# volume-em/empanada

Measured on AMD Instinct MI355X. Metric: Mvox/s end-to-end 3D panoptic inference (incl. consensus); PQ vs CPU ref, higher is better.
Workload: dtype f32

## Files before the change

empanada_amd/csrc/emp_wino4.hip:

```cpp
#include "emp_common.h"
#include "emp_wino4.h"
#include <stdlib.h>
#include <type_traits>

typedef float f32x4 __attribute__((ext_vector_type(4)));

#define WF_THREADS 512
#define WF_G 32
#define WF_S 16
#define WF_RS 34
#define WF_PS (WF_S * WF_RS)
#define WF_PF 3
#define WF_XCH (WF_THREADS * 48)
#define WF_T_MIN 3136

struct WfGeom {
    const float *x, *U, *scale, *shift;
    const int32_t *tiles;
    float *out;
    int64_t T, out_ps;
    int H, W, dil, groups;
};

template <int CIN, int COUT, bool RELU>
__global__ __launch_bounds__(WF_THREADS, 2) void wino4_fused_kernel(WfGeom g)
{
    constexpr int KS = CIN / WF_S;
    constexpr int CG = COUT / 64;
    __shared__ __attribute__((aligned(16))) float Vs[36 * WF_PS > WF_XCH ? 36 * WF_PS : WF_XCH];

    const int tid = threadIdx.x, wave = tid >> 6, lane = tid & 63;
    const int tl = tid >> 4, ch = tid & 15;
    const int ci = lane & 15, q = lane >> 4;
    const int odd = q >> 1;
    const int h = wave >> 2, w4 = wave & 3;

    const int xcd = blockIdx.x & 7, slot = blockIdx.x >> 3, per = gridDim.x >> 3;
    const int lo = (int)((int64_t)g.groups * xcd / 8), hi = (int)((int64_t)g.groups * (xcd + 1) / 8);
    const int n_items = slot < hi - lo ? ((hi - lo - slot + per - 1) / per) * CG : 0;

    auto load_raw = [&](int item, int s, v1 (&raw)[6][6]) -> int {
        const int64_t t = (int64_t)(lo + slot + (item / CG) * per) * WF_G + tl;
        const bool live = t < g.T;
        const int64_t tc = live ? t : g.T - 1;
        const int n = g.tiles[3 * tc], by = g.tiles[3 * tc + 1], bx = g.tiles[3 * tc + 2];
        const uint32_t src = 4u * ((uint32_t)n * (uint32_t)(g.H * g.W * CIN) + (uint32_t)(WF_S * s + ch));
        const char *xb = reinterpret_cast<const char *>(g.x);
        int mask = 0;
        uint32_t xo[6];
#pragma unroll
        for (int b = 0; b < 6; ++b) {
            const int xx = bx + b * g.dil;
            if (live && xx >= 0 && xx < g.W) mask |= 64 << b;
            xo[b] = 4u * (uint32_t)(min(max(xx, 0), g.W - 1) * CIN);
        }
#pragma unroll
        for (int a = 0; a < 6; ++a) {
            const int yy = by + a * g.dil;
            if (live && yy >= 0 && yy < g.H) mask |= 1 << a;
            const uint32_t row = src + 4u * (uint32_t)(min(max(yy, 0), g.H - 1) * (g.W * CIN));
#pragma unroll
            for (int b = 0; b < 6; ++b) raw[a][b] = {*reinterpret_cast<const float *>(xb + (row + xo[b]))};
        }
        return mask;
    };
    auto transform = [&](const v1 (&raw)[6][6], int mask) {
        v1 tt[6][6];
#pragma unroll
        for (int a = 0; a < 6; ++a) {
            v1 d[6];
#pragma unroll
            for (int b = 0; b < 6; ++b) d[b] = {(mask >> a & 1) && (mask >> (6 + b) & 1) ? raw[a][b].x : 0.f};
            wino4_bt(d, tt[a]);
        }
        float *dst = &Vs[ch * WF_RS + tl];
#pragma unroll
        for (int v = 0; v < 6; ++v) {
            v1 col[6], r[6];
#pragma unroll
            for (int a = 0; a < 6; ++a) col[a] = tt[a][v];
            wino4_bt(col, r);
#pragma unroll
            for (int u = 0; u < 6; ++u) dst[(u * 6 + v) * WF_PS] = r[u].x;
        }
    };

    const float *Al = &Vs[3 * h * WF_PS + (8 * (q & 1) + odd) * WF_RS + ci];
    const float *Ul = g.U + ((int64_t)3 * h * COUT + 16 * w4 + ci) * CIN + 8 * (q & 1) + 4 * odd;

    v1 raw[6][6];
    int mask = 0;
    if (n_items > 0) mask = load_raw(0, 0, raw);
    for (int item = 0; item < n_items; ++item) {
        const int cg = item % CG;
        f32x4 acc[18][2];
#pragma unroll
        for (int lp = 0; lp < 18; ++lp)
#pragma unroll
            for (int rt = 0; rt < 2; ++rt) acc[lp][rt] = {0.f, 0.f, 0.f, 0.f};

#pragma unroll 1
        for (int s = 0; s < KS; ++s) {
            transform(raw, mask);
            __syncthreads();
            const float *up = Ul + (int64_t)cg * 64 * CIN + WF_S * s;
            auto uoff = [](int lp) { return (int64_t)((lp / 3) * 6 + lp % 3) * COUT * CIN; };
            float4 bq[WF_PF];
#pragma unroll
            for (int lp = 0; lp < WF_PF; ++lp) bq[lp] = *reinterpret_cast<const float4 *>(up + uoff(lp));
            if (s + 1 < KS) mask = load_raw(item, s + 1, raw);
#pragma unroll
            for (int lp = 0; lp < 18; ++lp) {
                float4 c = bq[lp % WF_PF];
                asm volatile("" : "+v"(c.x), "+v"(c.y), "+v"(c.z), "+v"(c.w));
                if (lp + WF_PF < 18) bq[lp % WF_PF] = *reinterpret_cast<const float4 *>(up + uoff(lp + WF_PF));
                const auto s0 = __builtin_amdgcn_permlane32_swap(__float_as_uint(c.x), __float_as_uint(c.y), false, false);
                const auto s1 = __builtin_amdgcn_permlane32_swap(__float_as_uint(c.z), __float_as_uint(c.w), false, false);
                const float bv[4] = {__uint_as_float(s0[0]), __uint_as_float(s1[0]), __uint_as_float(s0[1]), __uint_as_float(s1[1])};
                const float *ap = Al + ((lp / 3) * 6 + lp % 3) * WF_PS;
#pragma unroll
                for (int j = 0; j < 4; ++j)
#pragma unroll
                    for (int rt = 0; rt < 2; ++rt)
                        acc[lp][rt] = __builtin_amdgcn_mfma_f32_16x16x4f32(ap[2 * j * WF_RS + 16 * rt], bv[j], acc[lp][rt], 0, 0, 0);
            }
            __syncthreads();
        }

        const int co = cg * 64 + 16 * w4 + ci;
        float keep[4][3][4];
        float *xw = &Vs[((wave ^ 4) * 48) * 64 + lane];
        const float *xr = &Vs[(wave * 48) * 64 + lane];
        auto rows = [&](auto rtc, auto sendc) {
            constexpr int rt = decltype(rtc)::value;
            constexpr bool send = decltype(sendc)::value;
#pragma unroll
            for (int bb = 0; bb < 3; ++bb)
#pragma unroll
                for (int r = 0; r < 4; ++r) {
                    v1 m[6], rr[4];
#pragma unroll
                    for (int a = 0; a < 6; ++a) m[a] = {acc[3 * a + bb][rt][r]};
                    wino4_at(m, rr);
#pragma unroll
                    for (int a = 0; a < 4; ++a) {
                        if (send) xw[((r * 3 + bb) * 4 + a) * 64] = rr[a].x;
                        else keep[r][bb][a] = rr[a].x;
                    }
                }
        };
        using std::integral_constant;
        if (h == 0) {
            rows(integral_constant<int, 1>(), integral_constant<bool, true>());
            rows(integral_constant<int, 0>(), integral_constant<bool, false>());
        } else {
            rows(integral_constant<int, 0>(), integral_constant<bool, true>());
            rows(integral_constant<int, 1>(), integral_constant<bool, false>());
        }
        if (item + 1 < n_items) mask = load_raw(item + 1, 0, raw);
        __syncthreads();

        const float sc = g.scale[co], sh = g.shift[co];
        const int64_t t0 = (int64_t)(lo + slot + (item / CG) * per) * WF_G + 16 * h + 4 * q;
#pragma unroll
        for (int r = 0; r < 4; ++r) {
            const int64_t t = t0 + r;
            if (t < g.T) {
                const int n = g.tiles[3 * t], oy = g.tiles[3 * t + 1] + g.dil, ox = g.tiles[3 * t + 2] + g.dil;
                float *dst = g.out + (int64_t)n * g.H * g.W * g.out_ps + co;
#pragma unroll
                for (int a = 0; a < 4; ++a) {
                    v1 sm[6], yv[4];
#pragma unroll
                    for (int bb = 0; bb < 3; ++bb) {
                        const float got = xr[((r * 3 + bb) * 4 + a) * 64];
                        sm[bb] = {h ? got : keep[r][bb][a]};
                        sm[3 + bb] = {h ? keep[r][bb][a] : got};
                    }
                    wino4_at(sm, yv);
#pragma unroll
                    for (int b = 0; b < 4; ++b) {
                        const int yy = oy + a * g.dil, xx = ox + b * g.dil;
                        if (yy < g.H && xx < g.W) {
                            float v = __fadd_rn(__fmul_rn(yv[b].x, sc), sh);
                            if (RELU) v = fmaxf(v, 0.f);
                            dst[((int64_t)yy * g.W + xx) * g.out_ps] = v;
                        }
                    }
                }
            }
        }
        __syncthreads();
    }
}

static bool wf_off()
{
    static const char *off = getenv("EMP_WINO4_NO_FUSED");
    return off && off[0] == '1';
}

static bool wf_shape_ok(int64_t T, int Cin, int Cout)
{
    return ((Cin == 64 && Cout == 64) || (Cin == 128 && Cout == 128)) && T > 0 && 16 * T * Cin < (1LL << 30) &&
           emp_conv_k_slab(T, Cout, 36, 0) == WF_S;
}

extern "C" int emp_wino4_fused_eligible(int64_t T, int Cin, int Cout, int has_scale_shift)
{
    if (wf_off() || !has_scale_shift) return 0;
    if (!(Cin == 64 && Cout == 64)) return 0;
    return wf_shape_ok(T, Cin, Cout) && T >= WF_T_MIN;
}

extern "C" int emp_wino4_conv_bn_act_nhwc(const float *x, int N, int H, int W, int Cin, int dil, const int32_t *tiles,
                                          int64_t T, const float *U, int Cout, const float *scale, const float *shift,
                                          int relu, float *out, int64_t out_pixel_stride, void *stream)
{
    EMP_REQUIRE(x && tiles && U && scale && shift && out, "wino4_conv: null pointer (scale and shift are required)");
    EMP_REQUIRE(N > 0 && H > 0 && W > 0 && dil >= 1 && T >= 0, "wino4_conv: bad shape");
    if (out_pixel_stride == 0) out_pixel_stride = Cout;
    EMP_REQUIRE(out_pixel_stride >= Cout, "wino4_conv: bad pixel stride");
    EMP_REQUIRE(((reinterpret_cast<uintptr_t>(x) | reinterpret_cast<uintptr_t>(U)) & 15) == 0 &&
                (reinterpret_cast<uintptr_t>(out) & 3) == 0, "wino4_conv: alignment");
    if (T == 0) return EMP_OK;
    EMP_REQUIRE(wf_shape_ok(T, Cin, Cout), "wino4_conv: 64 -> 64 or 128 -> 128 with the K-slab 16 plan only (T = %lld, %d -> %d)",
                (long long)T, Cin, Cout);
    EMP_REQUIRE((int64_t)N * H * W * Cin < (1LL << 30) && T < (1LL << 31) - WF_G, "wino4_conv: activation too large for 32-bit byte offsets");
    WfGeom g;
    g.x = x; g.U = U; g.scale = scale; g.shift = shift; g.tiles = tiles; g.out = out;
    g.T = T; g.out_ps = out_pixel_stride; g.H = H; g.W = W; g.dil = dil;
    g.groups = (int)emp_cdiv(T, WF_G);
    hipStream_t st = emp_stream(stream);
    const dim3 grid(256), block(WF_THREADS);
    if (Cin == 64) {
        if (relu) hipLaunchKernelGGL((wino4_fused_kernel<64, 64, true>), grid, block, 0, st, g);
        else hipLaunchKernelGGL((wino4_fused_kernel<64, 64, false>), grid, block, 0, st, g);
    } else {
        if (relu) hipLaunchKernelGGL((wino4_fused_kernel<128, 128, true>), grid, block, 0, st, g);
        else hipLaunchKernelGGL((wino4_fused_kernel<128, 128, false>), grid, block, 0, st, g);
    }
    EMP_CHECK_LAUNCH("emp_wino4_conv_bn_act_nhwc");
    return EMP_OK;
}
```

Baseline: 133.1.

## Stage Winograd input gathers through LDS with async global_load_lds and deeper U prefetch

Replaces the register-held raw input gather with global_load_lds_dword writes into a new LDS staging area, issued row by row during the MFMA loop of the previous slab. Filter (U) loads use inline-asm global_load_dwordx4 with a prefetch depth of 8 and explicit vmcnt waits computed per step, in place of the old depth-3 prefetch. Tile metadata and scale/shift loads for the epilogue and the next item are hoisted earlier, and one trailing barrier is removed. The aim is to hide global latency and cut register pressure, at the cost of a larger LDS footprint and fragile hand-counted vmcnt and m0 handling.

```diff
diff --git a/empanada_amd/csrc/emp_wino4.hip b/empanada_amd/csrc/emp_wino4.hip
--- a/empanada_amd/csrc/emp_wino4.hip
+++ b/empanada_amd/csrc/emp_wino4.hip
@@ -10,7 +10,8 @@
 #define WF_S 16
 #define WF_RS 34
 #define WF_PS (WF_S * WF_RS)
-#define WF_PF 3
+#define WF_UD 8
+#define WF_STG (WF_THREADS * 36)
 #define WF_XCH (WF_THREADS * 48)
 #define WF_T_MIN 3136
 
@@ -22,12 +23,59 @@
     int H, W, dil, groups;
 };
 
+__device__ __forceinline__ void wf_glds4(const char *sbase, uint32_t vrow, uint32_t vcol, unsigned lds_byte_addr)
+{
+    uint32_t voff;
+    asm volatile("v_add_u32 %0, %1, %2\n\ts_mov_b32 m0, %4\n\ts_nop 2\n\tglobal_load_lds_dword %0, %3"
+                 : "=&v"(voff) : "v"(vrow), "v"(vcol), "s"(sbase), "s"(lds_byte_addr) : "m0");
+}
+__device__ __forceinline__ f32x4 wf_ldu(const float *sbase, uint32_t voff)
+{
+    f32x4 r;
+    asm volatile("s_nop 4\n\tglobal_load_dwordx4 %0, %1, %2" : "=v"(r) : "v"(voff), "s"(sbase));
+    return r;
+}
+template <int N>
+__device__ __forceinline__ void wf_wait_u(f32x4 &c)
+{
+    asm volatile("s_waitcnt vmcnt(%1)" : "+v"(c) : "n"(N));
+}
+__device__ __forceinline__ void wf_wait_u(int n, f32x4 &c)
+{
+#define WF_W1(k) case k: wf_wait_u<k>(c); break;
+#define WF_W8(k) WF_W1(k) WF_W1(k + 1) WF_W1(k + 2) WF_W1(k + 3) WF_W1(k + 4) WF_W1(k + 5) WF_W1(k + 6) WF_W1(k + 7)
+    switch (n) {
+        WF_W8(0) WF_W8(8) WF_W8(16) WF_W8(24) WF_W8(32) WF_W8(40) WF_W8(48) WF_W8(56)
+        default: wf_wait_u<0>(c);
+    }
+#undef WF_W8
+#undef WF_W1
+}
+__device__ __forceinline__ void wf_wait_all()
+{
+    asm volatile("s_waitcnt vmcnt(0)" ::: "memory");
+}
+constexpr int wf_younger(int lp, bool gather)
+{
+    const int u = (lp + WF_UD - 1 < 17 ? lp + WF_UD - 1 : 17) - lp;
+    const int first = lp < WF_UD ? 0 : lp - WF_UD, last = lp - 1 < 5 ? lp - 1 : 5;
+    return u + (gather && last >= first ? 6 * (last - first + 1) : 0);
+}
+
 template <int CIN, int COUT, bool RELU>
 __global__ __launch_bounds__(WF_THREADS, 2) void wino4_fused_kernel(WfGeom g)
 {
     constexpr int KS = CIN / WF_S;
     constexpr int CG = COUT / 64;
-    __shared__ __attribute__((aligned(16))) float Vs[36 * WF_PS > WF_XCH ? 36 * WF_PS : WF_XCH];
+    static_assert(WF_XCH <= 36 * WF_PS + WF_STG && WF_UD >= 6 && WF_UD <= 18 && wf_younger(WF_UD, true) < 64, "LDS / vmcnt budget");
+    __shared__ __attribute__((aligned(16))) float Ls[WF_STG + 36 * WF_PS];
+    typedef __attribute__((address_space(3))) float lds_f;
+    auto fixed = [](float *p) {
+        unsigned a = (unsigned)(size_t)(lds_f *)p;
+        asm volatile("" : "+v"(a));
+        return (lds_f *)(size_t)a;
+    };
+    float *const Vs = Ls + WF_STG;
 
     const int tid = threadIdx.x, wave = tid >> 6, lane = tid & 63;
     const int tl = tid >> 4, ch = tid & 15;
@@ -39,41 +87,51 @@
     const int lo = (int)((int64_t)g.groups * xcd / 8), hi = (int)((int64_t)g.groups * (xcd + 1) / 8);
     const int n_items = slot < hi - lo ? ((hi - lo - slot + per - 1) / per) * CG : 0;
 
-    auto load_raw = [&](int item, int s, v1 (&raw)[6][6]) -> int {
-        const int64_t t = (int64_t)(lo + slot + (item / CG) * per) * WF_G + tl;
-        const bool live = t < g.T;
-        const int64_t tc = live ? t : g.T - 1;
-        const int n = g.tiles[3 * tc], by = g.tiles[3 * tc + 1], bx = g.tiles[3 * tc + 2];
-        const uint32_t src = 4u * ((uint32_t)n * (uint32_t)(g.H * g.W * CIN) + (uint32_t)(WF_S * s + ch));
-        const char *xb = reinterpret_cast<const char *>(g.x);
-        int mask = 0;
-        uint32_t xo[6];
+    uint32_t rowo[6], colo[6];
+    int mask = 0;
+    auto tile_geom = [&](int n, int by, int bx, bool live) {
+        const uint32_t src = 4u * ((uint32_t)n * (uint32_t)(g.H * g.W * CIN) + (uint32_t)ch);
+        mask = 0;
 #pragma unroll
         for (int b = 0; b < 6; ++b) {
             const int xx = bx + b * g.dil;
             if (live && xx >= 0 && xx < g.W) mask |= 64 << b;
-            xo[b] = 4u * (uint32_t)(min(max(xx, 0), g.W - 1) * CIN);
+            colo[b] = 4u * (uint32_t)(min(max(xx, 0), g.W - 1) * CIN);
         }
 #pragma unroll
         for (int a = 0; a < 6; ++a) {
             const int yy = by + a * g.dil;
             if (live && yy >= 0 && yy < g.H) mask |= 1 << a;
-            const uint32_t row = src + 4u * (uint32_t)(min(max(yy, 0), g.H - 1) * (g.W * CIN));
-#pragma unroll
-            for (int b = 0; b < 6; ++b) raw[a][b] = {*reinterpret_cast<const float *>(xb + (row + xo[b]))};
-        }
-        return mask;
-    };
-    auto transform = [&](const v1 (&raw)[6][6], int mask) {
+            rowo[a] = src + 4u * (uint32_t)(min(max(yy, 0), g.H - 1) * (g.W * CIN));
+        }
+    };
+    auto tile_index = [&](int item) -> int64_t {
+        const int64_t t = (int64_t)(lo + slot + (item / CG) * per) * WF_G + tl;
+        return t < g.T ? t : g.T - 1;
+    };
+    auto tile_live = [&](int item) { return (int64_t)(lo + slot + (item / CG) * per) * WF_G + tl < g.T; };
+    const unsigned lds0 = (unsigned)(size_t)(__attribute__((address_space(3))) float *)Ls;
+    const unsigned stg_dst = __builtin_amdgcn_readfirstlane(lds0 + (unsigned)(64 * wave * 4));
+    auto gather_row = [&](int a, int s) {
+        const char *xs = reinterpret_cast<const char *>(g.x) + 4 * WF_S * s;
+#pragma unroll
+        for (int b = 0; b < 6; ++b) wf_glds4(xs, rowo[a], colo[b], stg_dst + (unsigned)((a * 6 + b) * WF_THREADS * 4));
+    };
+    lds_f *const raw0 = fixed(&Ls[tid]), *const raw1 = fixed(&Ls[18 * WF_THREADS + tid]);
+    lds_f *const dst0 = fixed(&Vs[ch * WF_RS + tl]), *const dst1 = fixed(&Vs[18 * WF_PS + ch * WF_RS + tl]);
+    auto transform = [&]() {
         v1 tt[6][6];
 #pragma unroll
         for (int a = 0; a < 6; ++a) {
             v1 d[6];
-#pragma unroll
-            for (int b = 0; b < 6; ++b) d[b] = {(mask >> a & 1) && (mask >> (6 + b) & 1) ? raw[a][b].x : 0.f};
+            float val[6];
+#pragma unroll
+            for (int b = 0; b < 6; ++b) val[b] = (a < 3 ? raw0 : raw1)[((a % 3) * 6 + b) * WF_THREADS];
+            asm volatile("" : "+v"(val[0]), "+v"(val[1]), "+v"(val[2]), "+v"(val[3]), "+v"(val[4]), "+v"(val[5]));
+#pragma unroll
+            for (int b = 0; b < 6; ++b) d[b] = {(mask >> a & 1) && (mask >> (6 + b) & 1) ? val[b] : 0.f};
             wino4_bt(d, tt[a]);
         }
-        float *dst = &Vs[ch * WF_RS + tl];
 #pragma unroll
         for (int v = 0; v < 6; ++v) {
             v1 col[6], r[6];
@@ -81,16 +139,20 @@
             for (int a = 0; a < 6; ++a) col[a] = tt[a][v];
             wino4_bt(col, r);
 #pragma unroll
-            for (int u = 0; u < 6; ++u) dst[(u * 6 + v) * WF_PS] = r[u].x;
-        }
-    };
-
-    const float *Al = &Vs[3 * h * WF_PS + (8 * (q & 1) + odd) * WF_RS + ci];
-    const float *Ul = g.U + ((int64_t)3 * h * COUT + 16 * w4 + ci) * CIN + 8 * (q & 1) + 4 * odd;
-
-    v1 raw[6][6];
-    int mask = 0;
-    if (n_items > 0) mask = load_raw(0, 0, raw);
+            for (int u = 0; u < 6; ++u) (u < 3 ? dst0 : dst1)[((u % 3) * 6 + v) * WF_PS] = r[u].x;
+        }
+    };
+
+    lds_f *const Al0 = fixed(&Vs[3 * h * WF_PS + (8 * (q & 1) + odd) * WF_RS + ci]);
+    lds_f *const Al1 = fixed(&Vs[(18 + 3 * h) * WF_PS + (8 * (q & 1) + odd) * WF_RS + ci]);
+    const uint32_t uvo = 4u * (uint32_t)((3 * h * COUT + 16 * w4 + ci) * CIN + 8 * (q & 1) + 4 * odd);
+
+    if (n_items > 0) {
+        const int64_t tc = tile_index(0);
+        tile_geom(g.tiles[3 * tc], g.tiles[3 * tc + 1], g.tiles[3 * tc + 2], tile_live(0));
+#pragma unroll
+        for (int a = 0; a < 6; ++a) gather_row(a, 0);
+    }
     for (int item = 0; item < n_items; ++item) {
         const int cg = item % CG;
         f32x4 acc[18][2];
@@ -99,25 +161,26 @@
 #pragma unroll
             for (int rt = 0; rt < 2; ++rt) acc[lp][rt] = {0.f, 0.f, 0.f, 0.f};
 
-#pragma unroll 1
-        for (int s = 0; s < KS; ++s) {
-            transform(raw, mask);
+        auto slab = [&](int s, auto nextc) {
+            constexpr bool NEXT = decltype(nextc)::value;
+            wf_wait_all();
+            transform();
             __syncthreads();
-            const float *up = Ul + (int64_t)cg * 64 * CIN + WF_S * s;
-            auto uoff = [](int lp) { return (int64_t)((lp / 3) * 6 + lp % 3) * COUT * CIN; };
-            float4 bq[WF_PF];
-#pragma unroll
-            for (int lp = 0; lp < WF_PF; ++lp) bq[lp] = *reinterpret_cast<const float4 *>(up + uoff(lp));
-            if (s + 1 < KS) mask = load_raw(item, s + 1, raw);
+            const float *ub = g.U + (int64_t)cg * 64 * CIN + WF_S * s;
+            auto upos = [](int lp) { return (int64_t)((lp / 3) * 6 + lp % 3) * COUT * CIN; };
+            f32x4 bq[WF_UD];
+#pragma unroll
+            for (int lp = 0; lp < WF_UD; ++lp) bq[lp] = wf_ldu(ub + upos(lp), uvo);
 #pragma unroll
             for (int lp = 0; lp < 18; ++lp) {
-                float4 c = bq[lp % WF_PF];
-                asm volatile("" : "+v"(c.x), "+v"(c.y), "+v"(c.z), "+v"(c.w));
-                if (lp + WF_PF < 18) bq[lp % WF_PF] = *reinterpret_cast<const float4 *>(up + uoff(lp + WF_PF));
+                f32x4 c = bq[lp % WF_UD];
+                wf_wait_u(wf_younger(lp, NEXT), c);
+                if (lp + WF_UD < 18) bq[lp % WF_UD] = wf_ldu(ub + upos(lp + WF_UD), uvo);
+                if (NEXT && lp < 6) gather_row(lp, s + 1);
                 const auto s0 = __builtin_amdgcn_permlane32_swap(__float_as_uint(c.x), __float_as_uint(c.y), false, false);
                 const auto s1 = __builtin_amdgcn_permlane32_swap(__float_as_uint(c.z), __float_as_uint(c.w), false, false);
                 const float bv[4] = {__uint_as_float(s0[0]), __uint_as_float(s1[0]), __uint_as_float(s0[1]), __uint_as_float(s1[1])};
-                const float *ap = Al + ((lp / 3) * 6 + lp % 3) * WF_PS;
+                const lds_f *ap = (lp < 9 ? Al0 : Al1) + ((lp / 3 % 3) * 6 + lp % 3) * WF_PS;
 #pragma unroll
                 for (int j = 0; j < 4; ++j)
 #pragma unroll
@@ -125,12 +188,30 @@
                         acc[lp][rt] = __builtin_amdgcn_mfma_f32_16x16x4f32(ap[2 * j * WF_RS + 16 * rt], bv[j], acc[lp][rt], 0, 0, 0);
             }
             __syncthreads();
-        }
+        };
+        using std::integral_constant;
+#pragma unroll 1
+        for (int s = 0; s < KS - 1; ++s) slab(s, integral_constant<bool, true>());
+        slab(KS - 1, integral_constant<bool, false>());
 
         const int co = cg * 64 + 16 * w4 + ci;
+        const int64_t t0 = (int64_t)(lo + slot + (item / CG) * per) * WF_G + 16 * h + 4 * q;
+        const bool more = item + 1 < n_items, new_group = more && (item + 1) % CG == 0;
+        float sc, sh;
+        int on[4], oy[4], ox[4], nn, nby, nbx;
+        auto request = [&]() {
+            sc = g.scale[co], sh = g.shift[co];
+#pragma unroll
+            for (int r = 0; r < 4; ++r) {
+                const int64_t tc = t0 + r < g.T ? t0 + r : g.T - 1;
+                on[r] = g.tiles[3 * tc], oy[r] = g.tiles[3 * tc + 1], ox[r] = g.tiles[3 * tc + 2];
+            }
+            const int64_t tn = tile_index(item + 1);
+            nn = g.tiles[3 * tn], nby = g.tiles[3 * tn + 1], nbx = g.tiles[3 * tn + 2];
+        };
         float keep[4][3][4];
-        float *xw = &Vs[((wave ^ 4) * 48) * 64 + lane];
-        const float *xr = &Vs[(wave * 48) * 64 + lane];
+        float *xw = &Ls[((wave ^ 4) * 48) * 64 + lane];
+        const float *xr = &Ls[(wave * 48) * 64 + lane];
         auto rows = [&](auto rtc, auto sendc) {
             constexpr int rt = decltype(rtc)::value;
             constexpr bool send = decltype(sendc)::value;
@@ -149,38 +230,50 @@
                     }
                 }
         };
-        using std::integral_constant;
         if (h == 0) {
             rows(integral_constant<int, 1>(), integral_constant<bool, true>());
+            request();
             rows(integral_constant<int, 0>(), integral_constant<bool, false>());
         } else {
             rows(integral_constant<int, 0>(), integral_constant<bool, true>());
+            request();
             rows(integral_constant<int, 1>(), integral_constant<bool, false>());
         }
-        if (item + 1 < n_items) mask = load_raw(item + 1, 0, raw);
         __syncthreads();
-
-        const float sc = g.scale[co], sh = g.shift[co];
-        const int64_t t0 = (int64_t)(lo + slot + (item / CG) * per) * WF_G + 16 * h + 4 * q;
+        float got[4][3][4];
+#pragma unroll
+        for (int r = 0; r < 4; ++r)
+#pragma unroll
+            for (int bb = 0; bb < 3; ++bb)
+#pragma unroll
+                for (int a = 0; a < 4; ++a) got[r][bb][a] = xr[((r * 3 + bb) * 4 + a) * 64];
+        asm volatile("" : "+v"(sc), "+v"(sh), "+v"(nn), "+v"(nby), "+v"(nbx));
+#pragma unroll
+        for (int r = 0; r < 4; ++r) asm volatile("" : "+v"(on[r]), "+v"(oy[r]), "+v"(ox[r]));
+        __syncthreads();
+        if (more) {
+            if (new_group) tile_geom(nn, nby, nbx, tile_live(item + 1));
+#pragma unroll
+            for (int a = 0; a < 6; ++a) gather_row(a, 0);
+        }
+
 #pragma unroll
         for (int r = 0; r < 4; ++r) {
-            const int64_t t = t0 + r;
-            if (t < g.T) {
-                const int n = g.tiles[3 * t], oy = g.tiles[3 * t + 1] + g.dil, ox = g.tiles[3 * t + 2] + g.dil;
-                float *dst = g.out + (int64_t)n * g.H * g.W * g.out_ps + co;
+            if (t0 + r < g.T) {
+                const int oyy = oy[r] + g.dil, oxx = ox[r] + g.dil;
+                float *dst = g.out + (int64_t)on[r] * g.H * g.W * g.out_ps + co;
 #pragma unroll
                 for (int a = 0; a < 4; ++a) {
                     v1 sm[6], yv[4];
 #pragma unroll
                     for (int bb = 0; bb < 3; ++bb) {
-                        const float got = xr[((r * 3 + bb) * 4 + a) * 64];
-                        sm[bb] = {h ? got : keep[r][bb][a]};
-                        sm[3 + bb] = {h ? keep[r][bb][a] : got};
+                        sm[bb] = {h ? got[r][bb][a] : keep[r][bb][a]};
+                        sm[3 + bb] = {h ? keep[r][bb][a] : got[r][bb][a]};
                     }
                     wino4_at(sm, yv);
 #pragma unroll
                     for (int b = 0; b < 4; ++b) {
-                        const int yy = oy + a * g.dil, xx = ox + b * g.dil;
+                        const int yy = oyy + a * g.dil, xx = oxx + b * g.dil;
                         if (yy < g.H && xx < g.W) {
                             float v = __fadd_rn(__fmul_rn(yv[b].x, sc), sh);
                             if (RELU) v = fmaxf(v, 0.f);
@@ -190,8 +283,8 @@
                 }
             }
         }
-        __syncthreads();
     }
+    wf_wait_all();
 }
 
 static bool wf_off()
```

Result: no change. 132.9 (-0.2%).
